# mvenouziou/Boosted_DETR

Hardware: AMD Instinct MI355X
Metric: images/sec training step (fwd+matcher+loss+bwd), 640x640 N=100 (higher is better)
Workload: dtype f32 (conv/GEMM products as 3 split-f16 [fwd] / split-bf16 [grad] MFMA products, f32 accumulate)

## Files before the change

boosted_detr_amd/_lib.py:

```python
from __future__ import annotations

import ctypes as C
import os
from pathlib import Path

_LIB_PATH = Path(os.environ.get("BDETR_LIB") or Path(__file__).resolve().parent / "csrc" / "libbdetr.so")
_lib = None

c_f32p = C.c_void_p
c_i32p = C.c_void_p
c_i64p = C.c_void_p
c_stream = C.c_void_p


class ConvDesc(C.Structure):
    _fields_ = [(n, C.c_int) for n in ("N", "H", "W", "C", "K", "R", "S", "stride", "pad", "OH", "OW")]


class GemmDesc(C.Structure):
    _fields_ = [
        ("I", C.c_int), ("J", C.c_int), ("R", C.c_int), ("nb0", C.c_int), ("nb1", C.c_int),
        ("a", C.c_void_p), ("lda", C.c_int64), ("sa0", C.c_int64), ("sa1", C.c_int64), ("a_rcontig", C.c_int),
        ("b", C.c_void_p), ("ldb", C.c_int64), ("sb0", C.c_int64), ("sb1", C.c_int64), ("b_rcontig", C.c_int),
        ("c", C.c_void_p), ("ldc", C.c_int64), ("sc0", C.c_int64), ("sc1", C.c_int64),
# ... 60 lines not shown
    "bdetr_jpeg_quality_ws_bytes": (C.c_int64, [I, I, I]),
    "bdetr_jpeg_quality": (I, [P, P, P, I, I, I, P, P]),
    "bdetr_augment_jpeg": (I, [P, P, P, P, P, I, I, I, P, P, P]),
    "bdetr_conv2d_fwd": (I, [P, P, P, P, C.POINTER(ConvDesc), I, P, P, P]),
    "bdetr_conv2d_fwd_stat_chunks": (I, [C.POINTER(ConvDesc)]),
    "bdetr_conv2d_bwd_data": (I, [P, P, P, C.POINTER(ConvDesc), I, P]),
    "bdetr_conv2d_bwd_weight": (I, [P, P, P, C.POINTER(ConvDesc), I, P]),
    "bdetr_conv2d_bwd_weight_splitk": (I, [C.POINTER(ConvDesc)]),
    "bdetr_bn_apply_p16": (I, [P, P, P, P, P, P, I, C.POINTER(BnAffine), I, P, P, P, P, P, L, I, P]),
    "bdetr_bn_bwd_p16": (I, [P, P, I, P, P, P, P, P, I, I, P, P, P, P, P, P, P, P, I, L, I, P]),
    "bdetr_bn_bwd_p16_even_pixels": (I, [P, P, I, P, P, P, P, P, I, I, P, P, P, P, P, P, I, I, I, I, I, P]),
    "bdetr_p16_supported": (I, [C.POINTER(ConvDesc)]),
    "bdetr_p16_pack": (I, [P, L, P, P, P, P]),
    "bdetr_p16_unpack": (I, [P, I, L, P, P]),
    "bdetr_p16_pack_conv_weights": (I, [P, I, I, I, I, P, P, P, P]),
    "bdetr_p16_pack_conv_weights_multi": (I, [P, I, P, P]),
    "bdetr_p16_conv2d_fwd_stat_chunks": (I, [C.POINTER(ConvDesc)]),
    "bdetr_p16_conv2d_fwd": (I, [P, P, P, P, C.POINTER(ConvDesc), I, P, P, P]),
    "bdetr_p16_conv2d_bwd_data": (I, [P, P, P, C.POINTER(ConvDesc), I, P]),
    "bdetr_p16_conv2d_bwd_data_stat_chunks": (I, [C.POINTER(ConvDesc)]),
    "bdetr_p16_conv2d_bwd_data_masked_accum": (I, [P, P, P, P, C.POINTER(ConvDesc), C.POINTER(BnBwdFuse), P]),
    "bdetr_p16_conv2d_bwd_data_masked_accum_compact": (I, [P, P, P, P, P, C.POINTER(ConvDesc), C.POINTER(BnBwdFuse), P]),
    "bdetr_relu_mask_apply": (I, [P, P, C.c_int64, P]),
    "bdetr_p16_conv2d_bwd_data_bnstats": (I, [P, P, P, C.POINTER(ConvDesc), C.POINTER(BnBwdFuse), P]),
    "bdetr_p16_conv2d_bwd_weight_splitk": (I, [C.POINTER(ConvDesc)]),
    "bdetr_p16_conv2d_bwd_weight": (I, [P, P, P, C.POINTER(ConvDesc), I, P]),
    "bdetr_p16_conv2d_bwd_weight_xf16": (I, [P, P, P, C.POINTER(ConvDesc), I, P]),
    "bdetr_gemm": (I, [C.POINTER(GemmDesc), P]),
    "bdetr_gemm_ws": (I, [C.POINTER(GemmDesc), P, L, P]),
    "bdetr_splitk_workspace_elems": (L, [L, L, I]),
    "bdetr_conv2d_bwd_weight_ws": (I, [P, P, P, C.POINTER(ConvDesc), I, P, L, P]),
    "bdetr_p16_conv2d_bwd_weight_ws": (I, [P, I, P, P, C.POINTER(ConvDesc), I, P, L, P]),
    "bdetr_gemm_grouped": (I, [C.POINTER(GemmDesc), I, P]),
    "bdetr_colsum_chunks": (I, [L]),
    "bdetr_colsum": (I, [P, L, I, P, P, P]),
    "bdetr_colsum_accumulate": (I, [P, L, I, P, P]),
    "bdetr_colsum_accumulate_group": (I, [P, P, I, P, I, P]),
    "bdetr_colstats": (I, [P, L, I, P, P, P]),
    "bdetr_bn_stats": (I, [P, L, I, P, P, I, F, F, I, P, P, P, P, P, P, P]),
    "bdetr_flag_nonfinite": (I, [P, L, P, P]),
    "bdetr_flag_snapshot": (I, [P, P, P, I, P]),
    "bdetr_debug_checksum": (I, [P, L, P, P, P, I, U64, P]),
    "bdetr_graph_node_census": (I, [P, P, I]),
    "bdetr_bn_stats_fold_rows": (I, []),
    "bdetr_bn_stats_frozen": (I, [P, P, I, F, P, P, P]),
    "bdetr_bn_apply": (I, [P, P, P, P, P, P, I, P, L, I, P]),
    "bdetr_bn_bwd_chunks": (I, [L]),
    "bdetr_bn_bwd": (I, [P, P, P, P, P, P, P, I, I, P, P, P, P, P, L, I, P]),
    "bdetr_maxpool3x3s2_fwd": (I, [P, P, I, I, I, I, I, I, P]),
    "bdetr_maxpool3x3s2_bwd": (I, [P, P, P, P, I, I, I, I, I, I, P]),
    "bdetr_stem_pool_bwd_chunks": (I, [L]),
    "bdetr_stem_pool_fwd": (I, [P, P, P, P, P, I, I, I, I, P, P, P, P, P]),
    "bdetr_stem_pool_bwd": (I, [P, P, P, P, P, P, P, I, I, I, I, P, I, P, P, P, P]),
    "bdetr_p16_s2d_pack_bf16": (I, [P, I, I, I, P, P]),
    "bdetr_p16_stem_bwd_weight": (I, [P, P, P, I, I, I, I, P]),
    "bdetr_p16_s2d_unpack_dw": (I, [P, P, I, P]),
    "bdetr_attention_head_dim": (I, []),
    "bdetr_attention_fwd": (I, [P, P, P, P, P, I, I, I, I, F, P]),
    "bdetr_attention_bwd": (I, [P, P, P, P, P, P, P, P, P, P, I, I, I, I, F, P]),
    "bdetr_softmax_rows_fwd": (I, [P, P, L, I, F, P]),
    "bdetr_softmax_rows_bwd": (I, [P, P, P, L, I, F, P]),
    "bdetr_add_dropout_layernorm_fwd": (I, [P, P, P, P, P, P, P, L, I, F, F, U64, P, P]),
    "bdetr_ln_bwd_chunks": (I, [L]),
    "bdetr_add_dropout_layernorm_bwd": (I, [P, P, P, P, P, P, P, P, P, P, P, L, I, F, U64, P, I, P]),
    "bdetr_rowchain_fwd": (I, [C.POINTER(RowchainFwdDesc), P]),
    "bdetr_rowchain_bwd": (I, [C.POINTER(RowchainBwdDesc), P]),
# ... 74 lines not shown
```

boosted_detr_amd/csrc/igemm.hip:

```cpp
#include "gemm_common.h"
#include <stdlib.h>
#include <string.h>
#include <type_traits>
#include <utility>
#include <vector>

using namespace bdgemm;

namespace {

constexpr int BK = 32;
constexpr int RPAD = 4;
constexpr int NTHREADS = 256;

constexpr int SLD = 36;
constexpr int SLD3 = 52;
constexpr float LO_SCALE = 2048.f;
typedef __bf16 bf16x2 __attribute__((ext_vector_type(2)));
typedef __bf16 bf16x8 __attribute__((ext_vector_type(8)));
typedef _Float16 f16x2 __attribute__((ext_vector_type(2)));
typedef _Float16 f16x8 __attribute__((ext_vector_type(8)));
typedef float f32x2 __attribute__((ext_vector_type(2)));

template <int ARITH>
// ... 43 lines not shown
__device__ __forceinline__ f32x4 buf_load4(__amdgpu_buffer_rsrc_t r, unsigned byte_off) {
    return __builtin_bit_cast(f32x4, __builtin_amdgcn_raw_buffer_load_b128(r, (int)byte_off, 0, 0));
}
__device__ __forceinline__ float buf_load1(__amdgpu_buffer_rsrc_t r, unsigned byte_off) {
    return __builtin_bit_cast(float, __builtin_amdgcn_raw_buffer_load_b32(r, (int)byte_off, 0, 0));
}

template <int VEC>
struct DenseLoader {
    using Op = DenseOp;
    struct Ctx { unsigned off; bool ok; };
    static __device__ __forceinline__ const float* batch_base(const Op& op, int b0, int b1) {
        return op.p + (int64_t)b0 * op.s0 + (int64_t)b1 * op.s1;
    }
    static __device__ __forceinline__ void regroup(Op& op, const float* p, int x_extent, bool rc) {
        op.p = p;
        if (x_extent >= 0) { if (rc) op.rows = x_extent; else op.cols = x_extent; }
    }
    static __device__ __forceinline__ Ctx row_ctx(const Op& op, int row, int row_limit) {
        Ctx c; c.ok = row < row_limit; c.off = (unsigned)row * (unsigned)op.ld; return c;
    }
    static __device__ __forceinline__ f32x4 load(__amdgpu_buffer_rsrc_t rs, const Op& op, const Ctx& c, int col, int col_limit) {
        if (VEC == 4) {
            return buf_load4(rs, (c.ok && col < col_limit) ? (c.off + (unsigned)col) * 4u : OOB);
        } else {
            f32x4 v;
#pragma unroll
            for (int e = 0; e < 4; ++e) v[e] = buf_load1(rs, (c.ok && col + e < col_limit) ? (c.off + (unsigned)(col + e)) * 4u : OOB);
            return v;
        }
    }
};

struct PatchLoader {
    using Op = PatchOp;
    struct Ctx { int nbase; int ih0, iw0; bool ok; };
    static __device__ __forceinline__ const float* batch_base(const Op& op, int, int) { return op.p; }
    static __device__ __forceinline__ void regroup(Op&, const float*, int, bool) {}
    static __device__ __forceinline__ Ctx row_ctx(const Op& op, int row, int row_limit) {
        Ctx c; c.ok = row < row_limit;
        int ohw = op.OH * op.OW;
        int n = row / ohw; int rem = row - n * ohw;
        int oh = rem / op.OW; int ow = rem - oh * op.OW;
        c.nbase = n * op.H * op.W;
        c.ih0 = oh * op.stride - op.pad; c.iw0 = ow * op.stride - op.pad;
        return c;
    }
    static __device__ __forceinline__ f32x4 load(__amdgpu_buffer_rsrc_t rs, const Op& op, const Ctx& c, int col, int col_limit) {
        int tap = col / op.C; int ch = col - tap * op.C;
        int r = tap / op.S; int s = tap - r * op.S;
        int ih = c.ih0 + r, iw = c.iw0 + s;
        const bool ok = c.ok && col < col_limit && (unsigned)ih < (unsigned)op.H && (unsigned)iw < (unsigned)op.W;
        const unsigned off = ((unsigned)(c.nbase + ih * op.W + iw) * (unsigned)op.C + (unsigned)ch) * 4u;
        return buf_load4(rs, ok ? off : OOB);
    }
};

struct WFlipLoader {
    using Op = WFlipOp;
    struct Ctx { unsigned off; bool ok; };
    static __device__ __forceinline__ const float* batch_base(const Op& op, int, int) { return op.p; }
    static __device__ __forceinline__ void regroup(Op&, const float*, int, bool) {}
    static __device__ __forceinline__ Ctx row_ctx(const Op& op, int row, int row_limit) {
        Ctx c; c.ok = row < row_limit;
        int tap = row / op.K; int k = row - tap * op.K;
        int r = tap / op.S; int s = tap - r * op.S;
        c.off = (unsigned)(((k * op.R + (op.R - 1 - r)) * op.S + (op.S - 1 - s)) * op.C);
        return c;
    }
    static __device__ __forceinline__ f32x4 load(__amdgpu_buffer_rsrc_t rs, const Op& op, const Ctx& c, int col, int col_limit) {
        return buf_load4(rs, (c.ok && col < col_limit) ? (c.off + (unsigned)col) * 4u : OOB);
    }
};

template <int BX, bool RC>
struct TileGeom {
    static constexpr int LDS_FLOATS = RC ? BX * (BK + RPAD) : BK * BX;
    static constexpr int NV = BX * BK / 4 / NTHREADS;
    static constexpr int VPR = RC ? BK / 4 : BX / 4;
    static constexpr int LDS_LD = RC ? BK + RPAD : BX;
};

template <int BM, int BN, int WM, int WN, class LA, bool A_RC, class LB, bool B_RC, int ARITH>
__global__ __launch_bounds__(NTHREADS, 2)
void igemm_kernel(typename LA::Op opa, typename LB::Op opb, GemmParams g)
{
    static_assert(WM * WN == 4, "4 waves per workgroup");
    constexpr int WTM = BM / WM, WTN = BN / WN;
    constexpr int TM = WTM / 32, TN = WTN / 32;
    static_assert(TM >= 1 && TN >= 1, "wave tile must hold at least one 32x32 MFMA tile");
    using GA = TileGeom<BM, A_RC>;
    using GB = TileGeom<BN, B_RC>;
    static_assert(GA::NV >= 1 && GB::NV >= 1, "tile too small for 256 threads");

    constexpr bool SPLIT = ARITH != AR_FP32;
    constexpr bool X6 = ARITH == AR_BF16X6;
    constexpr int SLDK = X6 ? SLD3 : SLD;
    constexpr int A_FLOATS = SPLIT ? BM * SLDK : GA::LDS_FLOATS;
    constexpr int B_FLOATS = SPLIT ? BN * SLDK : GB::LDS_FLOATS;
    constexpr int STAGE_FLOATS = A_FLOATS + B_FLOATS;
    static_assert(!SPLIT || ((A_RC || GA::NV % 2 == 0) && (B_RC || GB::NV % 2 == 0)), "split mode transposes k-pairs");
    __shared__ __attribute__((aligned(16))) float lds[2 * STAGE_FLOATS];

    const int tid = threadIdx.x;
    const int lane = tid & 63;
    const int wave = tid >> 6;
    const int wm = wave / WN, wn = wave % WN;
    const int li = lane & 31, lh = lane >> 5;

    const int nwg_ = g.tiles_i * g.tiles_j;
    const bool sk_ = g.ngroups == 0 && g.splitk > 1;
    const int lin_ = sk_ ? xcd_tile(blockIdx.z * nwg_ + blockIdx.x, nwg_ * gridDim.z) : xcd_tile(blockIdx.x, nwg_);
    const int zz_ = sk_ ? lin_ / nwg_ : blockIdx.z;
    const int wg = sk_ ? lin_ - zz_ * nwg_ : lin_;
    const int tile_i = wg / g.tiles_j, tile_j = wg - tile_i * g.tiles_j;
    const int i0 = tile_i * BM, j0 = tile_j * BN;

    int b0 = 0, b1 = 0, r_begin = 0, r_end = g.R;
    if (g.ngroups > 0) {
        const int z = g.splitk > 1 ? (int)blockIdx.z / g.splitk : (int)blockIdx.z;
        if (g.splitk > 1) {
            r_begin = ((int)blockIdx.z - z * g.splitk) * g.r_chunk;
            r_end = min(g.R, r_begin + g.r_chunk);
        }
#define BDETR_PICK(arr) (z == 0 ? g.arr[0] : z == 1 ? g.arr[1] : z == 2 ? g.arr[2] : g.arr[3])
        g.I = BDETR_PICK(gI); g.c = BDETR_PICK(gc); g.bias = BDETR_PICK(gbias);
        const float* pa = BDETR_PICK(ga);
        const float* pb = BDETR_PICK(gb);
#undef BDETR_PICK
        if (i0 >= g.I) return;
        LA::regroup(opa, pa, g.I, A_RC);
        LB::regroup(opb, pb, -1, B_RC);
    } else if (g.splitk > 1) {
        r_begin = zz_ * g.r_chunk;
        r_end = min(g.R, r_begin + g.r_chunk);
    } else {
        b0 = blockIdx.z / g.nb1; b1 = blockIdx.z - b0 * g.nb1;
    }
    const __amdgpu_buffer_rsrc_t rsA = make_rsrc(LA::batch_base(opa, b0, b1));
    const __amdgpu_buffer_rsrc_t rsB = make_rsrc(LB::batch_base(opb, b0, b1));
    const int a_rows = A_RC ? opa.rows : min(opa.rows, r_end), a_cols = A_RC ? min(opa.cols, r_end) : opa.cols;
    const int b_rows = B_RC ? opb.rows : min(opb.rows, r_end), b_cols = B_RC ? min(opb.cols, r_end) : opb.cols;

    typename LA::Ctx ctxA[GA::NV];
    typename LB::Ctx ctxB[GB::NV];
    int colA[GA::NV], colB[GB::NV], ldsoffA[GA::NV], ldsoffB[GB::NV], rowA[GA::NV], rowB[GB::NV];
    auto stage_geom = [&](int p, int vpr, int bx, bool rc, int lds_ld, int& row, int& col, int& ldsoff) {
        if (!SPLIT) {
            const int v = tid + NTHREADS * p;
            const int rt = v / vpr, c4 = v - rt * vpr;
            row = rt; col = 4 * c4; ldsoff = rt * lds_ld + 4 * c4;
        } else if (rc) {
            const int v = tid + NTHREADS * p;
            const int q = v / vpr, c4 = v - q * vpr;
            const int rt = (q & ~15) | ((q & 3) << 2) | ((q >> 2) & 3);
            row = rt; col = 4 * c4;
            ldsoff = rt * SLDK * 32 + ((((c4 >> 1) ^ ((rt >> 4) & 7)) << 2) | ((c4 & 1) << 1));
        } else {
            const int u = tid + NTHREADS * (p >> 1);
            const int kp = u / (bx / 4), c4 = u - kp * (bx / 4);
            row = 2 * kp + (p & 1); col = 4 * c4;
            ldsoff = (4 * c4) * SLDK * 32 + ((((kp >> 2) ^ ((c4 >> 2) & 7)) << 2) | (kp & 3));
        }
    };
#pragma unroll
    for (int p = 0; p < GA::NV; ++p) {
        stage_geom(p, GA::VPR, BM, A_RC, GA::LDS_LD, rowA[p], colA[p], ldsoffA[p]);
        if (A_RC) ctxA[p] = LA::row_ctx(opa, i0 + rowA[p], a_rows);
    }
#pragma unroll
    for (int p = 0; p < GB::NV; ++p) {
        stage_geom(p, GB::VPR, BN, B_RC, GB::LDS_LD, rowB[p], colB[p], ldsoffB[p]);
        if (B_RC) ctxB[p] = LB::row_ctx(opb, j0 + rowB[p], b_rows);
    }

    f32x4 stA0[GA::NV], stB0[GB::NV], stA1[GA::NV], stB1[GB::NV];
    auto load_stage = [&](int r0, f32x4 (&ra)[GA::NV], f32x4 (&rb)[GB::NV]) {
#pragma unroll
        for (int p = 0; p < GA::NV; ++p) {
            if (A_RC) ra[p] = LA::load(rsA, opa, ctxA[p], r0 + colA[p], a_cols);
            else      ra[p] = LA::load(rsA, opa, LA::row_ctx(opa, r0 + rowA[p], a_rows), i0 + colA[p], a_cols);
        }
#pragma unroll
        for (int p = 0; p < GB::NV; ++p) {
            if (B_RC) rb[p] = LB::load(rsB, opb, ctxB[p], r0 + colB[p], b_cols);
            else      rb[p] = LB::load(rsB, opb, LB::row_ctx(opb, r0 + rowB[p], b_rows), j0 + colB[p], b_cols);
        }
    };
    auto write_split = [&](unsigned* base, bool rc, auto nv_c, const f32x4* r, const int* ldsoff) {
        constexpr int nv = decltype(nv_c)::value;
        if (rc) {
#pragma unroll
            for (int p = 0; p < nv; ++p) {
                unsigned* row = base + (ldsoff[p] >> 5);
                const int w = ldsoff[p] & 31;
                if constexpr (X6) {
                    unsigned h0, m0, l0, h1, m1, l1;
                    split3(r[p][0], r[p][1], h0, m0, l0);
                    split3(r[p][2], r[p][3], h1, m1, l1);
                    u32x2 hi, mid, lo;
                    hi[0] = h0; hi[1] = h1; mid[0] = m0; mid[1] = m1; lo[0] = l0; lo[1] = l1;
                    *reinterpret_cast<u32x2*>(row + w) = hi;
                    *reinterpret_cast<u32x2*>(row + (w ^ 16)) = mid;
                    *reinterpret_cast<u32x2*>(row + 32 + (w & 15)) = lo;
                } else {
                    unsigned h0, l0, h1, l1;
                    split2<ARITH>(r[p][0], r[p][1], h0, l0);
                    split2<ARITH>(r[p][2], r[p][3], h1, l1);
                    u32x2 hi, lo;
                    hi[0] = h0; hi[1] = h1; lo[0] = l0; lo[1] = l1;
                    *reinterpret_cast<u32x2*>(row + w) = hi;
                    *reinterpret_cast<u32x2*>(row + (w ^ 16)) = lo;
                }
            }
        } else {
#pragma unroll
            for (int p = 0; p + 1 < nv; p += 2) {
                unsigned* row = base + (ldsoff[p] >> 5);
                const int w = ldsoff[p] & 31;
// ... 235 lines not shown
    }
    if (tiles(128, 128) >= 16LL * num_cus() && J >= 1024) return {128, 128};
    return {64, 64};
}

struct ProfRec { hipEvent_t e0, e1; double flops; int I, J, R, z, bm, bn, kind; };
std::vector<ProfRec> g_prof_recs;
std::vector<std::pair<hipEvent_t, hipEvent_t>> g_prof_pool;
size_t g_prof_used = 0;

template <class L> struct LoaderId { static constexpr int v = 0; };
template <> struct LoaderId<PatchLoader> { static constexpr int v = 1; };
template <> struct LoaderId<WFlipLoader> { static constexpr int v = 2; };
template <> struct LoaderId<DenseLoader<1>> { static constexpr int v = 3; };

}
namespace bdgemm {
bool g_prof_on = false;
void prof_begin(hipStream_t st, double flops, int I, int J, int R, int z, int bm, int bn, int kind) {
    if (g_prof_used == g_prof_pool.size()) {
        hipEvent_t a, b;
        if (hipEventCreate(&a) != hipSuccess || hipEventCreate(&b) != hipSuccess) return;
        g_prof_pool.emplace_back(a, b);
    }
    auto& ev = g_prof_pool[g_prof_used++];
    g_prof_recs.push_back({ev.first, ev.second, flops, I, J, R, z, bm, bn, kind});
    (void)hipEventRecord(ev.first, st);
}
void prof_end(hipStream_t st) { (void)hipEventRecord(g_prof_recs.back().e1, st); }
}
namespace {

template <int BM, int BN, int WM, int WN, class LA, bool A_RC, class LB, bool B_RC, int ARITH = AR_FP32>
int launch_cfg(const typename LA::Op& a, const typename LB::Op& b, GemmParams g, int zdim, hipStream_t st) {
    g.tiles_i = (int)cdiv64(g.I, BM);
    g.tiles_j = (int)cdiv64(g.J, BN);
    dim3 grid(g.tiles_i * g.tiles_j, 1, zdim);
    g.vec_store = (g.J % 4 == 0) && (g.ldc % 4 == 0) && (g.sc0 % 4 == 0) && (g.sc1 % 4 == 0) && ((reinterpret_cast<uintptr_t>(g.c) & 15) == 0);
    const bool prof = g_prof_on;
    if (prof) prof_begin(st, 2.0 * (double)g.I * (double)g.J * (double)g.R * (g.splitk > 1 ? (g.ngroups > 0 ? (double)g.ngroups : 1.0) : (double)zdim), g.I, g.J, g.R, zdim, BM, BN,
                         ARITH * 10000 + LoaderId<LA>::v * 1000 + (A_RC ? 100 : 0) + LoaderId<LB>::v * 10 + (B_RC ? 1 : 0));
    hipLaunchKernelGGL((igemm_kernel<BM, BN, WM, WN, LA, A_RC, LB, B_RC, ARITH>), grid, dim3(NTHREADS), 0, st, a, b, g);
    if (prof) prof_end(st);
    return bdetr_launch_status("igemm");
}

template <class LA, bool A_RC, class LB, bool B_RC>
int launch_any(const typename LA::Op& a, const typename LB::Op& b, GemmParams g, int zdim, hipStream_t st, int arith, bool small_only = false) {
    if (arith == AR_FP16X3 && !(A_RC && B_RC)) arith = AR_FP32;
    constexpr bool PATCH = LoaderId<LA>::v == 1 || LoaderId<LB>::v == 1;
    TileChoice t = small_only ? TileChoice{64, 64} : choose_tile(g.I, g.J, g.splitk > 1 ? 2 : zdim, A_RC && B_RC, arith != AR_FP32, PATCH);
    if constexpr (LoaderId<LA>::v != 3 && LoaderId<LB>::v != 3) {
        if (arith == AR_BF16X3 && t.bn >= 64) {
            if (t.bm == 128 && t.bn == 128) return launch_cfg<128, 128, 2, 2, LA, A_RC, LB, B_RC, AR_BF16X3>(a, b, g, zdim, st);
            if (t.bm == 128 && t.bn == 64)  return launch_cfg<128, 64, 2, 2, LA, A_RC, LB, B_RC, AR_BF16X3>(a, b, g, zdim, st);
            return launch_cfg<64, 64, 2, 2, LA, A_RC, LB, B_RC, AR_BF16X3>(a, b, g, zdim, st);
        }
        if (arith == AR_BF16X6 && t.bn >= 64) {
            if (t.bm == 128) return launch_cfg<128, 64, 2, 2, LA, A_RC, LB, B_RC, AR_BF16X6>(a, b, g, zdim, st);
            return launch_cfg<64, 64, 2, 2, LA, A_RC, LB, B_RC, AR_BF16X6>(a, b, g, zdim, st);
        }
        if constexpr (A_RC && B_RC) {
            if (arith == AR_FP16X3 && t.bn >= 64) {
                if (t.bm == 128 && t.bn == 128) return launch_cfg<128, 128, 2, 2, LA, A_RC, LB, B_RC, AR_FP16X3>(a, b, g, zdim, st);
                if (t.bm == 128 && t.bn == 64)  return launch_cfg<128, 64, 2, 2, LA, A_RC, LB, B_RC, AR_FP16X3>(a, b, g, zdim, st);
                return launch_cfg<64, 64, 2, 2, LA, A_RC, LB, B_RC, AR_FP16X3>(a, b, g, zdim, st);
            }
        }
    }
    if (t.bm == 128 && t.bn == 128) return launch_cfg<128, 128, 2, 2, LA, A_RC, LB, B_RC>(a, b, g, zdim, st);
    if (t.bm == 128 && t.bn == 64)  return launch_cfg<128, 64, 2, 2, LA, A_RC, LB, B_RC>(a, b, g, zdim, st);
    if (t.bm == 128 && t.bn == 32)  return launch_cfg<128, 32, 4, 1, LA, A_RC, LB, B_RC>(a, b, g, zdim, st);
    return launch_cfg<64, 64, 2, 2, LA, A_RC, LB, B_RC>(a, b, g, zdim, st);
// ... 105 lines not shown
        BDETR_CHECK_ARG(span_ok((int64_t)(e.a_rcontig ? e.I : e.R) * e.lda) && span_ok((int64_t)(e.b_rcontig ? e.J : e.R) * e.ldb),
                        "bdetr_gemm_grouped: operand %d spans 4 GB or more (32-bit buffer offsets)", k);
        g.ga[k] = e.a; g.gb[k] = e.b; g.gc[k] = e.c; g.gbias[k] = e.bias; g.gI[k] = e.I;
        if (e.I > maxI) maxI = e.I;
        v4 = v4 && aligned16(e.a) && aligned16(e.b) && aligned16(e.c);
    }
    const bdetr_gemm_desc& f = d[0];
    bool dims4 = f.J % 4 == 0 && (f.a_rcontig || f.b_rcontig ? f.R % 4 == 0 : true);
    for (int k = 0; k < n; ++k) dims4 = dims4 && (f.a_rcontig || d[k].I % 4 == 0);
    BDETR_CHECK_ARG(v4 && f.lda % 4 == 0 && f.ldb % 4 == 0 && f.ldc % 4 == 0 && dims4,
                    "bdetr_gemm_grouped: operands must be 16-byte aligned with contiguous dimensions that are multiples of 4");
    g.ngroups = n;
    g.I = maxI; g.J = f.J; g.R = f.R;
    g.c = f.c; g.ldc = f.ldc; g.bias = f.bias; g.alpha = f.alpha; g.act = f.act;
    g.mode = f.accumulate ? ST_ACCUM : ST_STORE;
    int zdim = n;
    if (f.splitk > 1) {
        g.r_chunk = (int)(cdiv64(cdiv64(f.R, f.splitk), BK) * BK);
        g.splitk = (int)cdiv64(f.R, g.r_chunk);
        g.mode = ST_ATOMIC;
        zdim = n * g.splitk;
    }
    DenseOp a{f.a, f.lda, 0, 0, f.a_rcontig ? maxI : f.R, f.a_rcontig ? f.R : maxI};
    DenseOp b{f.b, f.ldb, 0, 0, f.b_rcontig ? f.J : f.R, f.b_rcontig ? f.R : f.J};
    hipStream_t st = (hipStream_t)stream;
    const bool arc = f.a_rcontig != 0, brc = f.b_rcontig != 0;
    const int sp = use_split(f.grad != 0);
    if (arc && brc)   return launch_any<DenseLoader<4>, true, DenseLoader<4>, true>(a, b, g, zdim, st, sp);
    if (arc && !brc)  return launch_any<DenseLoader<4>, true, DenseLoader<4>, false>(a, b, g, zdim, st, sp);
    if (!arc && !brc) return launch_any<DenseLoader<4>, false, DenseLoader<4>, false>(a, b, g, zdim, st, sp);
    return launch_any<DenseLoader<4>, false, DenseLoader<4>, true>(a, b, g, zdim, st, sp, true);
}

extern "C" int bdetr_gemm(const bdetr_gemm_desc* d, void* stream) { return bdetr_gemm_ws(d, nullptr, 0, stream); }

template <class F>
static int with_splitk_slabs(GemmParams& g, int zdim, float* ws, int64_t ws_elems, hipStream_t st, const char* who, F&& launch) {
    float* c = g.c;
    const int64_t n = (int64_t)g.I * g.J, slab = splitk_slab(n);
    BDETR_CHECK_ARG(g.ldc == g.J, "%s: the split-K workspace form needs a dense C (ldc == J)", who);
    BDETR_CHECK_ARG(aligned16(ws) && ws_elems >= (int64_t)zdim * slab, "%s: workspace too small or misaligned (%lld floats, need %lld)", who,
                    (long long)ws_elems, (long long)((int64_t)zdim * slab));
    g.c = ws; g.sc0 = slab; g.mode = ST_STORE;
    if (int e = launch()) return e;
    return splitk_fold(ws, zdim, slab, c, n, st);
}

extern "C" int bdetr_gemm_ws(const bdetr_gemm_desc* d, float* ws, int64_t ws_elems, void* stream) {
    BDETR_CHECK_ARG(d && d->a && d->b && d->c, "bdetr_gemm: null pointer");
    BDETR_CHECK_ARG(d->I > 0 && d->J > 0 && d->R >= 0, "bdetr_gemm: bad shape I=%d J=%d R=%d", d->I, d->J, d->R);
    const int nb0 = d->nb0 > 0 ? d->nb0 : 1, nb1 = d->nb1 > 0 ? d->nb1 : 1;
    const int splitk = d->splitk > 1 ? d->splitk : 1;
    BDETR_CHECK_ARG(splitk == 1 || (nb0 * nb1 == 1 && !d->bias && d->act == 0), "bdetr_gemm: splitk needs a single plain GEMM");
    hipStream_t st = (hipStream_t)stream;

    DenseOp a{d->a, d->lda, d->sa0, d->sa1, d->a_rcontig ? d->I : d->R, d->a_rcontig ? d->R : d->I};
    DenseOp b{d->b, d->ldb, d->sb0, d->sb1, d->b_rcontig ? d->J : d->R, d->b_rcontig ? d->R : d->J};
    BDETR_CHECK_ARG(span_ok(dense_span(a)) && span_ok(dense_span(b)),
                    "bdetr_gemm: an operand matrix spans 4 GB or more (32-bit buffer offsets); split the problem");
    GemmParams g; init_params(g);
    g.I = d->I; g.J = d->J; g.R = d->R; g.nb1 = nb1;
    g.c = d->c; g.ldc = d->ldc; g.sc0 = d->sc0; g.sc1 = d->sc1;
    g.bias = d->bias; g.alpha = d->alpha; g.act = d->act;
    g.mode = splitk > 1 ? ST_ATOMIC : (d->accumulate ? ST_ACCUM : ST_STORE);
    int zdim = nb0 * nb1;
    if (splitk > 1) {
// ... 162 lines not shown
```

boosted_detr_amd/engine.py:

```python
from __future__ import annotations

import math
import zlib
from typing import Callable, Dict, List, Optional, Sequence

import numpy as np
import torch

from . import kernels as K

_DEVICE = None


def device() -> torch.device:
    global _DEVICE
    if _DEVICE is None:
        if not torch.cuda.is_available():
            raise RuntimeError("boosted_detr_amd needs an AMD GPU (HIP device); there is no CPU execution path")
        _DEVICE = torch.device("cuda", torch.cuda.current_device())
    return _DEVICE


def to_device(a, dtype=torch.float32) -> torch.Tensor:
    if isinstance(a, torch.Tensor):
# ... 176 lines not shown
        K.relu_mask_apply_(g, r.lazy_mask)
        r.lazy_mask = None
    return g


class Tape:

    def __init__(self):
        self.nodes: List[tuple] = []

    def record(self, outputs: Sequence[torch.Tensor], inputs: Sequence[Optional[torch.Tensor]], fn: Callable) -> None:
        self.nodes.append((tuple(outputs), tuple(inputs), fn))

    def backward(self, seeds: Dict[int, torch.Tensor]) -> Dict[int, torch.Tensor]:
        grads: Dict[int, torch.Tensor] = dict(seeds)
        for outputs, inputs, fn in reversed(self.nodes):
            gouts = [grads.pop(id(o), None) for o in outputs]
            if all(g is None for g in gouts):
                continue
            if not getattr(fn, "accepts_lazy", False):
                gouts = [materialise(g) for g in gouts]
            acc = None
            if getattr(fn, "wants_acc", False):
                acc = []
                for t in inputs:
                    have = grads.get(id(t)) if t is not None else None
                    acc.append(have if info(have).owned else None)
                gins = fn(*gouts, acc=acc)
            else:
                gins = fn(*gouts)
            if not isinstance(gins, (tuple, list)):
                gins = (gins,)
            assert len(gins) == len(inputs), (len(gins), len(inputs))
            for i, (t, g) in enumerate(zip(inputs, gins)):
                if t is None or g is None:
                    continue
                key = id(t)
                if key in grads:
                    if acc is not None and acc[i] is not None and g is acc[i]:
                        grads[key] = g
                        continue
                    g, have = materialise(g), materialise(grads[key])
                    dense_contribution(have)
                    if info(have).owned:
                        K.axpy_(1.0, g.view(have.shape), have)
                        grads[key] = have
                    else:
                        grads[key] = own(K.add(have, g.view(have.shape)))
                else:
                    grads[key] = g
            if _CAPTURE[0] is not None:
                _CAPTURE[0].maybe_cut(next((g for g in gins if isinstance(g, torch.Tensor)), None) if _DEBUG_LOG[0] is not None else None)
            elif _DEBUG_LOG[0] is not None and _DEBUG_LOG[0].eager_pending >= SegmentedCapture.SIDE_TASKS_PER_SEGMENT:
                _debug_cut(next((g for g in gins if isinstance(g, torch.Tensor)), None))
        return grads


_TAPE: Optional[Tape] = None
_CAPTURE = [None]


def capture() -> Optional["SegmentedCapture"]:
    return _CAPTURE[0]


def set_capture(cap: Optional["SegmentedCapture"]) -> None:
    _CAPTURE[0] = cap

import os as _os

# ... 451 lines not shown
```

boosted_detr_amd/kernels.py:

```python
from __future__ import annotations

import ctypes as C
from dataclasses import dataclass
from typing import Optional, Tuple

import numpy as np
import torch

from . import _lib
from ._lib import BnAffine, BnBwdFuse, ConvDesc, GemmDesc, LossDesc, RowchainBwdDesc, RowchainFwdDesc, check

ACT_NONE, ACT_RELU, ACT_TANH = 0, 1, 2


_LAUNCH_STREAM = [None]


def set_launch_stream(handle: Optional[int]) -> Optional[int]:
    prev = _LAUNCH_STREAM[0]
    _LAUNCH_STREAM[0] = handle
    return prev


GEMM_FP32, GEMM_BF16X3, GEMM_MIXED, GEMM_SPLIT, GEMM_BF16X6 = 0, 1, 2, 3, 4
# ... 423 lines not shown
def gemm_raw(I, J, R, a, lda, a_rc, b, ldb, b_rc, c, ldc, *, nb0=1, nb1=1, sa=(0, 0), sb=(0, 0), sc=(0, 0),
             bias=None, alpha=1.0, act=ACT_NONE, accumulate=False, splitk=1, grad=False):
    _chk(a, b, c, bias)
    g = GemmDesc(I, J, R, nb0, nb1, _p(a), lda, sa[0], sa[1], int(a_rc), _p(b), ldb, sb[0], sb[1], int(b_rc),
                 _p(c), ldc, sc[0], sc[1], _p(bias), float(alpha), act, int(accumulate), splitk, int(grad))
    ws, n = _splitk_ws(I, J, splitk, c) if ldc == J else (None, 0)
    check(_lib.lib().bdetr_gemm_ws(C.byref(g), _p(ws), n, _stream()), "gemm")
    return c


def gemm_grouped(descs):
    arr = (GemmDesc * len(descs))()
    for k, (I, J, R, a, lda, a_rc, b, ldb, b_rc, c, ldc, bias, act, acc) in enumerate(descs):
        _chk(a, b, c, bias)
        arr[k] = GemmDesc(I, J, R, 1, 1, _p(a), lda, 0, 0, int(a_rc), _p(b), ldb, 0, 0, int(b_rc), _p(c), ldc, 0, 0, _p(bias), 1.0, act,
                          int(acc), 1, int(not (a_rc and b_rc)))
    check(_lib.lib().bdetr_gemm_grouped(arr, len(descs), _stream()), "gemm_grouped")


def linear_fwd_group(xs, ws, biases, act=ACT_NONE):
    K_, O = xs[0].shape[1], ws[0].shape[0]
    ys = [empty(x.shape[0], O, like=x) for x in xs]
    gemm_grouped([(x.shape[0], O, K_, x, K_, True, w, K_, True, y, O, b, act, False) for x, w, b, y in zip(xs, ws, biases, ys)])
    return ys


def linear_bwd_data_group(dys, ws):
    O, K_ = ws[0].shape
    dxs = [empty(dy.shape[0], K_, like=dy) for dy in dys]
    gemm_grouped([(dy.shape[0], K_, O, dy, O, True, w, K_, False, dx, K_, None, ACT_NONE, False) for dy, w, dx in zip(dys, ws, dxs)])
    return dxs


def linear_fwd(x2d, w, bias, act=ACT_NONE):
    M, K = x2d.shape
    O = w.shape[0]
    y = empty(M, O, like=x2d)
    return gemm_raw(M, O, K, x2d, K, True, w, K, True, y, O, bias=bias, act=act)


def linear_bwd_data(dy2d, w, dx=None, accumulate=False):
    M, O = dy2d.shape
    K = w.shape[1]
    if dx is None:
        dx = empty(M, K, like=dy2d)
    return gemm_raw(M, K, O, dy2d, O, True, w, K, False, dx, K, accumulate=accumulate, grad=True)


def _auto_splitk(I, J, R) -> int:
    cus = _lib.lib().bdetr_device_cus()
    tiles = max(1, ((I + 63) // 64) * ((J + 63) // 64))
    sk = max(1, min((2 * cus) // tiles, R // 128))
    return sk


def linear_bwd_weight(dy2d, x2d, dw=None, prezeroed: bool = False):
    M, O = dy2d.shape
    K = x2d.shape[1]
    if dw is None:
        dw = empty(O, K, like=dy2d)
        prezeroed = False
    sk = _auto_splitk(O, K, M)
    if sk > 1 and not prezeroed:
        check(_lib.lib().bdetr_zero(_p(dw), dw.numel(), _stream()), "zero")
    return gemm_raw(O, K, M, dy2d, O, False, x2d, K, False, dw, K, splitk=sk, grad=True)

# ... 513 lines not shown
```

boosted_detr_amd/ops.py:

```python
from __future__ import annotations

import math
import os
import weakref
from typing import Optional

import numpy as np
import torch

from . import kernels as K
from . import _lib
from .engine import WEIGHTS_VERSION, Variable, current_tape, dense_contribution, info, materialise, own, side_task, tag

_dropout_site = [0]
_dropout_seed_dev = [None]


def dropout_seed_tensor() -> torch.Tensor:
    if _dropout_seed_dev[0] is None:
        _dropout_seed_dev[0] = torch.full((1,), 0x5EED, dtype=torch.int64, device="cuda")
    return _dropout_seed_dev[0]


def set_dropout_seed(seed: int, write: bool = True) -> None:
# ... 472 lines not shown
            _param_grads_task(w, b, lambda dw, pz: K.stem_bwd_weight_s2d(x32, dy, dw), None, x32, dy)
        else:
            _param_grads_task(w, b, lambda dw, pz: K.conv2d_bwd_weight(x32, dy, g, dw=dw, prezeroed=pz), None, x32, dy)
        return (None,)

    _rec([out], [x], backward)
    return out


def dense(x: torch.Tensor, w: Variable, b: Variable, act: int = K.ACT_NONE) -> torch.Tensor:
    x2d = _2d(x)
    y2d = K.linear_fwd(x2d, w.value, b.value, act)
    y = y2d.view(*x.shape[:-1], w.value.shape[0])

    def backward(g_out, acc=None):
        g2d = _2d(g_out.contiguous())
        if act == K.ACT_RELU:
            g2d = K.relu_bwd(y2d, g2d)
        elif act == K.ACT_TANH:
            g2d = K.tanh_bwd(y2d, g2d)
        _param_grads_task(w, b, lambda dw, pz: K.linear_bwd_weight(g2d, x2d, dw=dw, prezeroed=pz), g2d, x2d, g2d)
        have = acc[0] if acc is not None else None
        if have is not None and have.is_contiguous() and have.shape == x.shape:
            K.linear_bwd_data(g2d, w.value, dx=_2d(materialise(have)), accumulate=True)
            dense_contribution(have)
            return (have,)
        return (own(K.linear_bwd_data(g2d, w.value).view(x.shape)),)

    backward.wants_acc = True
    _rec([y], [x], backward)
    return y


def dense_group(xs, ws, bs):
    x2 = [_2d(x) for x in xs]
    aligned = all(t.data_ptr() % 16 == 0 for t in x2) and x2[0].shape[1] % 4 == 0 and ws[0].value.shape[0] % 4 == 0
    same = all(w.value.shape == ws[0].value.shape for w in ws)
    if not (aligned and same) or len(xs) > 4:
        return [dense(x, w, b) for x, w, b in zip(xs, ws, bs)]
    y2 = K.linear_fwd_group(x2, [w.value for w in ws], [b.value for b in bs])
    ys = [y.view(*x.shape[:-1], y.shape[1]) for y, x in zip(y2, xs)]

    def backward(*gs):
        g2 = [_2d(g.contiguous()) for g in gs]

        def param_grads():
            groups = {}
            for g, x, w in zip(g2, x2, ws):
                if w.needs_grad:
                    groups.setdefault((tuple(g.shape), tuple(x.shape)), []).append((g, x, GradSink(w)))
            for members in groups.values():
                K.linear_bwd_weight_group([m[0] for m in members], [m[1] for m in members], [m[2].buf for m in members], [m[2].mode == "direct" for m in members])
                for m in members:
                    m[2].commit()
            sinks = [(g, GradSink(b)) for g, b in zip(g2, bs) if b.needs_grad]
            direct = [(g, s) for g, s in sinks if s.mode == "direct"]
            if len(direct) > 1 and not K.deterministic() and all(g.shape[1] == direct[0][0].shape[1] for g, _ in direct):
                K.colsum_group([g for g, _ in direct], [s.buf for _, s in direct])
                for _, s in direct:
                    s.commit()
                sinks = [(g, s) for g, s in sinks if s.mode != "direct"]
            for g, s in sinks:
                K.colsum(g, out=s.buf, prezeroed=s.mode == "direct")
                s.commit()
        if any(w.needs_grad or b.needs_grad for w, b in zip(ws, bs)):
            side_task(param_grads, *x2, *g2)
        dxs = K.linear_bwd_data_group(g2, [w.value for w in ws])
        return tuple(own(dx.view(x.shape)) for dx, x in zip(dxs, xs))

    _rec(ys, list(xs), backward)
    return ys


def add(a: torch.Tensor, b: torch.Tensor) -> torch.Tensor:
    out = K.add(a, b)
    _rec([out], [a, b], lambda g: (g, g))
    return out


def _param_or_tensor_grad(p, fn):
    if isinstance(p, Variable):
        if p.needs_grad:
            s = GradSink(p)
            fn(s.buf)
            s.commit()
        return None
    return fn(None)


def add_bcast(x: torch.Tensor, row) -> torch.Tensor:
    rv = row.value if isinstance(row, Variable) else row
    out = K.add_bcast_rows(x, rv)
    n = rv.numel()

    def backward(g):
        g = g.contiguous()
        grow = _param_or_tensor_grad(row, lambda out_: K.sum_over_batch(g, n, out=out_))
        return g, (grow.view(rv.shape) if grow is not None else None)

    _rec([out], [x, None if isinstance(row, Variable) else row], backward)
    return out

# ... 193 lines not shown
```

include/bdetr.h:

```cpp
#ifndef BDETR_H
#define BDETR_H
#include <stdint.h>
#ifdef __cplusplus
extern "C" {
#endif

#define BDETR_ABI_VERSION 8

int         bdetr_abi_version(void);
const char* bdetr_last_error(void);
int         bdetr_device_cus(void);

int         bdetr_low_priority_stream_create(void** stream_out);
int         bdetr_stream_priority_range(int* least, int* greatest);
int         bdetr_side_stream_candidates(void* main_stream, int ncand, int loads, int ticks, void** streams_out, float* scores_ms, float* unloaded_ms);
int         bdetr_stream_destroy(void* stream);

enum { BDETR_GEMM_FP32 = 0, BDETR_GEMM_BF16X3 = 1, BDETR_GEMM_MIXED = 2, BDETR_GEMM_SPLIT = 3, BDETR_GEMM_BF16X6 = 4 };
int         bdetr_set_gemm_precision(int mode);
int         bdetr_get_gemm_precision(void);

int bdetr_prof_enable(int on);
int bdetr_prof_read(double* total_ms, int64_t* launches, double* flops);
int bdetr_prof_read_arith(int arith, double* total_ms, int64_t* launches, double* flops);
// ... 62 lines not shown
    const float* y; const float* mean; const float* rstd; const float* gamma; const float* beta; int relu;
    float* part_g; float* part_gx;
    const uint64_t* relu_mask;
    const float* y2; const float* mean2; const float* rstd2; float* part_gx2;
} bdetr_bn_bwd_fuse;
int bdetr_p16_conv2d_bwd_data_stat_chunks(const bdetr_conv_desc* d);
int bdetr_relu_mask_apply(float* x, const uint64_t* relu_mask, int64_t n, void* stream);
int bdetr_p16_conv2d_bwd_data_masked_accum(const void* dy_bf16, const void* wt_bf16, float* dx, const uint64_t* relu_mask,
                                           const bdetr_conv_desc* d, const bdetr_bn_bwd_fuse* bn , void* stream);
int bdetr_p16_conv2d_bwd_data_masked_accum_compact(const void* dy_bf16, const void* wt_bf16, float* dx, const float* old_even,
                                                   const uint64_t* relu_mask, const bdetr_conv_desc* d, const bdetr_bn_bwd_fuse* bn, void* stream);
int bdetr_p16_conv2d_bwd_data_bnstats(const void* dy_bf16, const void* wt_bf16, float* dx,
                                      const bdetr_conv_desc* d, const bdetr_bn_bwd_fuse* bn, void* stream);
int bdetr_p16_conv2d_bwd_weight_splitk(const bdetr_conv_desc* d);
int bdetr_p16_conv2d_bwd_weight(const void* x_bf16, const void* dy_bf16, float* dw,
                                const bdetr_conv_desc* d, int splitk, void* stream);
int bdetr_p16_conv2d_bwd_weight_xf16(const void* x_f16, const void* dy_bf16, float* dw,
                                     const bdetr_conv_desc* d, int splitk, void* stream);
int bdetr_p16_conv2d_bwd_weight_ws(const void* x, int x_is_f16, const void* dy_bf16, float* dw,
                                   const bdetr_conv_desc* d, int splitk, float* ws, int64_t ws_elems, void* stream);

typedef struct {
    int I, J, R;
    int nb0, nb1;
    const float* a; int64_t lda, sa0, sa1; int a_rcontig;
    const float* b; int64_t ldb, sb0, sb1; int b_rcontig;
    float*       c; int64_t ldc, sc0, sc1;
    const float* bias; float alpha; int act; int accumulate; int splitk;
    int grad;
} bdetr_gemm_desc;
int bdetr_gemm(const bdetr_gemm_desc* g, void* stream);
int bdetr_gemm_ws(const bdetr_gemm_desc* g, float* ws, int64_t ws_elems, void* stream);
int bdetr_gemm_grouped(const bdetr_gemm_desc* g, int n, void* stream);

int bdetr_colsum_chunks(int64_t rows);
int bdetr_colsum(const float* x, int64_t rows, int cols, float* out, float* ws, void* stream);
int bdetr_colsum_accumulate(const float* x, int64_t rows, int cols, float* out, void* stream);
int bdetr_colsum_accumulate_group(const float* const* xs, const int64_t* rows, int cols, float* const* outs, int n, void* stream);

int bdetr_colstats(const float* x, int64_t rows, int C, float* part_sum, float* part_sq, void* stream);
int bdetr_bn_stats(const float* x, int64_t rows, int C, const float* part_sum, const float* part_sq,
                   int nparts, float eps, float momentum, int bessel,
                   float* mean, float* rstd, float* moving_mean, float* moving_var, float* fold_ws,
                   int* guard_flag, void* stream);
int bdetr_flag_nonfinite(const float* x, int64_t n, int* flag, void* stream);
int bdetr_flag_snapshot(const int* flag, int* ordinal, int* host_ring, int ring_len, void* stream);
int bdetr_debug_checksum(const float* x, int64_t n, uint64_t* scratch, uint64_t* log, int* cursor, int cap, uint64_t tag, void* stream);
int bdetr_graph_node_census(void* graph, int64_t* counts, int ncounts);
int bdetr_bn_stats_fold_rows(void);
int bdetr_bn_stats_frozen(const float* moving_mean, const float* moving_var, int C, float eps,
                          float* mean, float* rstd, void* stream);
int bdetr_bn_apply(const float* x, const float* mean, const float* rstd, const float* gamma,
                   const float* beta, const float* residual, int relu, float* out,
                   int64_t rows, int C, void* stream);
int bdetr_bn_bwd_chunks(int64_t rows);
int bdetr_bn_bwd(const float* dout, const float* out, const float* x, const float* mean,
                 const float* rstd, const float* gamma, const float* beta, int relu, int frozen,
                 float* dx, float* dgamma, float* dbeta, float* dresidual,
                 float* ws, int64_t rows, int C, void* stream);

int bdetr_maxpool3x3s2_fwd(const float* x, float* y, int N, int H, int W, int C, int OH, int OW, void* stream);
int bdetr_maxpool3x3s2_bwd(const float* x, const float* y, const float* dy, float* dx,
                           int N, int H, int W, int C, int OH, int OW, void* stream);

int bdetr_stem_pool_bwd_chunks(int64_t rows);
int bdetr_stem_pool_fwd(const float* y, const float* mean, const float* rstd, const float* gamma, const float* beta,
// ... 128 lines not shown
```

Measured before the change: 649.0.

## Fuse fan-in linear backward-data products into one K-chained GEMM per destination

Adds a K-chained GEMM loader that walks several (dy, W) pairs in sequence inside one kernel, so the input gradients of a dense group whose members share an input are summed in the accumulator. The result can also be written straight into an existing gradient buffer. This removes the separate per-member backward-data GEMMs, the intermediate dx tensors and the elementwise gradient additions done by the autograd engine. The engine learns to skip re-adding aliased gradients the backward has already summed. It adds complexity in the GEMM kernel and the autograd path, and is bypassed in deterministic mode.

```diff
diff --git a/boosted_detr_amd/_lib.py b/boosted_detr_amd/_lib.py
--- a/boosted_detr_amd/_lib.py
+++ b/boosted_detr_amd/_lib.py
@@ -116,6 +116,7 @@
     "bdetr_conv2d_bwd_weight_ws": (I, [P, P, P, C.POINTER(ConvDesc), I, P, L, P]),
     "bdetr_p16_conv2d_bwd_weight_ws": (I, [P, I, P, P, C.POINTER(ConvDesc), I, P, L, P]),
     "bdetr_gemm_grouped": (I, [C.POINTER(GemmDesc), I, P]),
+    "bdetr_linear_bwd_data_fanin": (I, [P, P, P, P, I, I, I, I, I, P]),
     "bdetr_colsum_chunks": (I, [L]),
     "bdetr_colsum": (I, [P, L, I, P, P, P]),
     "bdetr_colsum_accumulate": (I, [P, L, I, P, P]),
diff --git a/boosted_detr_amd/csrc/igemm.hip b/boosted_detr_amd/csrc/igemm.hip
--- a/boosted_detr_amd/csrc/igemm.hip
+++ b/boosted_detr_amd/csrc/igemm.hip
@@ -99,6 +99,27 @@
     }
 };
 
+constexpr int CHAIN_MAX = 12;
+struct ChainOp { const float* p[CHAIN_MAX]; int64_t ld; int rows, cols; int n[2], rm, acc; };
+struct ChainLoader {
+    using Op = ChainOp;
+    using Ctx = DenseLoader<4>::Ctx;
+    static constexpr bool CHAINED = true;
+    static __device__ __forceinline__ const float* member(const Op& op, int m) { return op.p[m]; }
+    static __device__ __forceinline__ int first(const Op& op, int z) { return z == 0 ? 0 : op.n[0]; }
+    static __device__ __forceinline__ int count(const Op& op, int z) { return z == 0 ? op.n[0] : op.n[1]; }
+    static __device__ __forceinline__ const float* batch_base(const Op& op, int z, int) { return op.p[first(op, z)]; }
+    static __device__ __forceinline__ void regroup(Op&, const float*, int, bool) {}
+    static __device__ __forceinline__ Ctx row_ctx(const Op& op, int row, int row_limit) {
+        Ctx c; c.ok = row < row_limit; c.off = (unsigned)row * (unsigned)op.ld; return c;
+    }
+    static __device__ __forceinline__ f32x4 load(__amdgpu_buffer_rsrc_t rs, const Op&, const Ctx& c, int col, int col_limit) {
+        return buf_load4(rs, (c.ok && col < col_limit) ? (c.off + (unsigned)col) * 4u : OOB);
+    }
+};
+template <class L, class = void> struct IsChained { static constexpr bool v = false; };
+template <class L> struct IsChained<L, std::enable_if_t<L::CHAINED>> { static constexpr bool v = true; };
+
 struct PatchLoader {
     using Op = PatchOp;
     struct Ctx { int nbase; int ih0, iw0; bool ok; };
@@ -162,6 +183,8 @@
 
     constexpr bool SPLIT = ARITH != AR_FP32;
     constexpr bool X6 = ARITH == AR_BF16X6;
+    constexpr bool CHAIN = IsChained<LA>::v;
+    static_assert(CHAIN == IsChained<LB>::v, "both operands of a K-chained product are chained");
     constexpr int SLDK = X6 ? SLD3 : SLD;
     constexpr int A_FLOATS = SPLIT ? BM * SLDK : GA::LDS_FLOATS;
     constexpr int B_FLOATS = SPLIT ? BN * SLDK : GB::LDS_FLOATS;
@@ -204,8 +227,16 @@
     } else {
         b0 = blockIdx.z / g.nb1; b1 = blockIdx.z - b0 * g.nb1;
     }
-    const __amdgpu_buffer_rsrc_t rsA = make_rsrc(LA::batch_base(opa, b0, b1));
-    const __amdgpu_buffer_rsrc_t rsB = make_rsrc(LB::batch_base(opb, b0, b1));
+    __amdgpu_buffer_rsrc_t rsA = make_rsrc(LA::batch_base(opa, b0, b1));
+    __amdgpu_buffer_rsrc_t rsB = make_rsrc(LB::batch_base(opb, b0, b1));
+    [[maybe_unused]] int ch_m = 0, ch_r = 0;
+    [[maybe_unused]] int ch_n = 1, ch_first = 0;
+    if constexpr (CHAIN) {
+        g.c = b0 == 0 ? g.gc[0] : g.gc[1];
+        g.mode = ((opa.acc >> b0) & 1) ? ST_ACCUM : ST_STORE;
+        ch_n = LA::count(opa, b0); ch_first = LA::first(opa, b0);
+        r_end = ch_n * opa.rm;
+    }
     const int a_rows = A_RC ? opa.rows : min(opa.rows, r_end), a_cols = A_RC ? min(opa.cols, r_end) : opa.cols;
     const int b_rows = B_RC ? opb.rows : min(opb.rows, r_end), b_cols = B_RC ? min(opb.cols, r_end) : opb.cols;
 
@@ -243,6 +274,7 @@
 
     f32x4 stA0[GA::NV], stB0[GB::NV], stA1[GA::NV], stB1[GB::NV];
     auto load_stage = [&](int r0, f32x4 (&ra)[GA::NV], f32x4 (&rb)[GB::NV]) {
+        if constexpr (CHAIN) r0 = ch_r;
 #pragma unroll
         for (int p = 0; p < GA::NV; ++p) {
             if (A_RC) ra[p] = LA::load(rsA, opa, ctxA[p], r0 + colA[p], a_cols);
@@ -252,6 +284,14 @@
         for (int p = 0; p < GB::NV; ++p) {
             if (B_RC) rb[p] = LB::load(rsB, opb, ctxB[p], r0 + colB[p], b_cols);
             else      rb[p] = LB::load(rsB, opb, LB::row_ctx(opb, r0 + rowB[p], b_rows), j0 + colB[p], b_cols);
+        }
+        if constexpr (CHAIN) {
+            ch_r += BK;
+            if (ch_r >= opa.rm && ch_m + 1 < ch_n) {
+                ++ch_m; ch_r = 0;
+                rsA = make_rsrc(LA::member(opa, ch_first + ch_m));
+                rsB = make_rsrc(LB::member(opb, ch_first + ch_m));
+            }
         }
     };
     auto write_split = [&](unsigned* base, bool rc, auto nv_c, const f32x4* r, const int* ldsoff) {
@@ -553,13 +593,14 @@
 namespace {
 
 template <int BM, int BN, int WM, int WN, class LA, bool A_RC, class LB, bool B_RC, int ARITH = AR_FP32>
-int launch_cfg(const typename LA::Op& a, const typename LB::Op& b, GemmParams g, int zdim, hipStream_t st) {
+int launch_cfg(const typename LA::Op& a, const typename LB::Op& b, GemmParams g, int zdim, hipStream_t st, double prof_flops = -1.0, int prof_R = 0) {
     g.tiles_i = (int)cdiv64(g.I, BM);
     g.tiles_j = (int)cdiv64(g.J, BN);
     dim3 grid(g.tiles_i * g.tiles_j, 1, zdim);
     g.vec_store = (g.J % 4 == 0) && (g.ldc % 4 == 0) && (g.sc0 % 4 == 0) && (g.sc1 % 4 == 0) && ((reinterpret_cast<uintptr_t>(g.c) & 15) == 0);
     const bool prof = g_prof_on;
-    if (prof) prof_begin(st, 2.0 * (double)g.I * (double)g.J * (double)g.R * (g.splitk > 1 ? (g.ngroups > 0 ? (double)g.ngroups : 1.0) : (double)zdim), g.I, g.J, g.R, zdim, BM, BN,
+    if (prof && prof_flops >= 0.0) prof_begin(st, prof_flops, g.I, g.J, prof_R, 1, BM, BN, ARITH * 10000 + (A_RC ? 100 : 0) + (B_RC ? 1 : 0));
+    else if (prof) prof_begin(st, 2.0 * (double)g.I * (double)g.J * (double)g.R * (g.splitk > 1 ? (g.ngroups > 0 ? (double)g.ngroups : 1.0) : (double)zdim), g.I, g.J, g.R, zdim, BM, BN,
                          ARITH * 10000 + LoaderId<LA>::v * 1000 + (A_RC ? 100 : 0) + LoaderId<LB>::v * 10 + (B_RC ? 1 : 0));
     hipLaunchKernelGGL((igemm_kernel<BM, BN, WM, WN, LA, A_RC, LB, B_RC, ARITH>), grid, dim3(NTHREADS), 0, st, a, b, g);
     if (prof) prof_end(st);
@@ -731,6 +772,45 @@
     return launch_any<DenseLoader<4>, false, DenseLoader<4>, true>(a, b, g, zdim, st, sp, true);
 }
 
+extern "C" int bdetr_linear_bwd_data_fanin(const float* const* gs, const float* const* ws, float* const* dxs, const int* nmem, int ndst,
+                                           int I, int J, int R, int acc_bits, void* stream) {
+    BDETR_CHECK_ARG(gs && ws && dxs && nmem && ndst >= 1 && ndst <= 2, "bdetr_linear_bwd_data_fanin: 1..2 destinations");
+    int total = 0, longest = 0;
+    for (int z = 0; z < ndst; ++z) {
+        BDETR_CHECK_ARG(nmem[z] >= 1 && nmem[z] <= 6, "bdetr_linear_bwd_data_fanin: destination %d has %d members (1..6)", z, nmem[z]);
+        total += nmem[z];
+        if (nmem[z] > longest) longest = nmem[z];
+    }
+    static_assert(CHAIN_MAX >= 2 * 6, "two destinations of six members");
+    BDETR_CHECK_ARG(I > 0 && J > 0 && R > 0 && J % 4 == 0 && R % BK == 0,
+                    "bdetr_linear_bwd_data_fanin: bad shape I=%d J=%d R=%d (J a multiple of 4, R a multiple of %d)", I, J, R, BK);
+    BDETR_CHECK_ARG(span_ok((int64_t)I * R) && span_ok((int64_t)R * J),
+                    "bdetr_linear_bwd_data_fanin: an operand spans 4 GB or more (32-bit buffer offsets)");
+    ChainOp a{}, b{};
+    for (int k = 0; k < total; ++k) {
+        BDETR_CHECK_ARG(gs[k] && ws[k] && aligned16(gs[k]) && aligned16(ws[k]), "bdetr_linear_bwd_data_fanin: member %d is null or not 16-byte aligned", k);
+        a.p[k] = gs[k]; b.p[k] = ws[k];
+    }
+    GemmParams g; init_params(g);
+    for (int z = 0; z < ndst; ++z) {
+        BDETR_CHECK_ARG(dxs[z] && aligned16(dxs[z]), "bdetr_linear_bwd_data_fanin: destination %d is null or not 16-byte aligned", z);
+        g.gc[z] = dxs[z];
+        a.n[z] = b.n[z] = nmem[z];
+    }
+    a.ld = R; a.rows = I; a.cols = R; a.rm = R; a.acc = acc_bits;
+    b.ld = J; b.rows = R; b.cols = J; b.rm = R; b.acc = acc_bits;
+    g.I = I; g.J = J; g.R = longest * R;
+    g.c = dxs[0]; g.ldc = J;
+    hipStream_t st = (hipStream_t)stream;
+    const double flops = 2.0 * (double)I * (double)J * (double)R * (double)total;
+    if (J <= 32) return launch_cfg<128, 32, 4, 1, ChainLoader, true, ChainLoader, false>(a, b, g, ndst, st, flops, total * R);
+    switch (use_split(true)) {
+        case AR_BF16X3: return launch_cfg<64, 64, 2, 2, ChainLoader, true, ChainLoader, false, AR_BF16X3>(a, b, g, ndst, st, flops, total * R);
+        case AR_BF16X6: return launch_cfg<64, 64, 2, 2, ChainLoader, true, ChainLoader, false, AR_BF16X6>(a, b, g, ndst, st, flops, total * R);
+        default:        return launch_cfg<64, 64, 2, 2, ChainLoader, true, ChainLoader, false>(a, b, g, ndst, st, flops, total * R);
+    }
+}
+
 extern "C" int bdetr_gemm(const bdetr_gemm_desc* d, void* stream) { return bdetr_gemm_ws(d, nullptr, 0, stream); }
 
 template <class F>
diff --git a/boosted_detr_amd/engine.py b/boosted_detr_amd/engine.py
--- a/boosted_detr_amd/engine.py
+++ b/boosted_detr_amd/engine.py
@@ -232,10 +232,15 @@
             if not isinstance(gins, (tuple, list)):
                 gins = (gins,)
             assert len(gins) == len(inputs), (len(gins), len(inputs))
+            summed = {} if getattr(fn, "sums_aliases", False) else None
             for i, (t, g) in enumerate(zip(inputs, gins)):
                 if t is None or g is None:
                     continue
                 key = id(t)
+                if summed is not None:
+                    if summed.get(key) is g:
+                        continue
+                    summed[key] = g
                 if key in grads:
                     if acc is not None and acc[i] is not None and g is acc[i]:
                         grads[key] = g
diff --git a/boosted_detr_amd/kernels.py b/boosted_detr_amd/kernels.py
--- a/boosted_detr_amd/kernels.py
+++ b/boosted_detr_amd/kernels.py
@@ -479,6 +479,33 @@
     return dxs
 
 
+FANIN_MAX_MEMBERS, FANIN_MAX_DESTS = 6, 2
+
+
+def fanin_applies(dys, ws) -> bool:
+    O, K_ = ws[0].shape
+    return (O % 32 == 0 and K_ % 4 == 0 and all(w.shape == ws[0].shape and w.is_contiguous() and w.data_ptr() % 16 == 0 for w in ws)
+            and all(dy.shape == dys[0].shape and dy.is_contiguous() and dy.data_ptr() % 16 == 0 for dy in dys))
+
+
+def linear_bwd_data_fanin(dests):
+    assert 1 <= len(dests) <= FANIN_MAX_DESTS and all(1 <= len(d[0]) <= FANIN_MAX_MEMBERS and len(d[0]) == len(d[1]) for d in dests)
+    M, O = dests[0][0][0].shape
+    K_ = dests[0][1][0].shape[1]
+    gs = [g for d in dests for g in d[0]]
+    ws = [w for d in dests for w in d[1]]
+    assert all(g.shape == (M, O) for g in gs) and all(w.shape == (O, K_) for w in ws)
+    assert all(d[2] is not None or not d[3] for d in dests)
+    dxs = [d[2] if d[2] is not None else empty(M, K_, like=gs[0]) for d in dests]
+    assert all(dx.shape == (M, K_) for dx in dxs)
+    _chk(*gs, *ws, *dxs)
+    PA, PD, NA = C.c_void_p * len(gs), C.c_void_p * len(dxs), C.c_int * len(dxs)
+    acc_bits = sum(1 << z for z, d in enumerate(dests) if d[3])
+    check(_lib.lib().bdetr_linear_bwd_data_fanin(PA(*[g.data_ptr() for g in gs]), PA(*[w.data_ptr() for w in ws]), PD(*[dx.data_ptr() for dx in dxs]),
+                                                 NA(*[len(d[0]) for d in dests]), len(dxs), M, K_, O, acc_bits, _stream()), "linear_bwd_data_fanin")
+    return dxs
+
+
 def linear_fwd(x2d, w, bias, act=ACT_NONE):
     M, K = x2d.shape
     O = w.shape[0]
diff --git a/boosted_detr_amd/ops.py b/boosted_detr_amd/ops.py
--- a/boosted_detr_amd/ops.py
+++ b/boosted_detr_amd/ops.py
@@ -528,6 +528,44 @@
     return y
 
 
+FANIN = os.environ.get("BDETR_FANIN", "1") != "0"
+
+
+def _dense_group_fanin(xs, g2, wv, acc):
+    if not FANIN or K.deterministic() or not K.fanin_applies(g2[:1], wv):
+        return None
+    dests = {}
+    for i, x in enumerate(xs):
+        d = dests.setdefault(id(x), [[], None])
+        d[0].append(i)
+        have = acc[i] if acc is not None else None
+        if have is not None and have.is_contiguous() and have.shape == x.shape and info(have).compact_even is None:
+            d[1] = have
+    if len(dests) == len(xs) and all(d[1] is None for d in dests.values()):
+        return None
+    by_rows = {}
+    for d in dests.values():
+        if len(d[0]) > K.FANIN_MAX_MEMBERS or not K.fanin_applies([g2[i] for i in d[0]], wv):
+            return None
+        by_rows.setdefault(g2[d[0][0]].shape[0], []).append(d)
+    out = [None] * len(xs)
+    for group in by_rows.values():
+        for k in range(0, len(group), K.FANIN_MAX_DESTS):
+            part = group[k:k + K.FANIN_MAX_DESTS]
+            haves = [None if d[1] is None else materialise(d[1]) for d in part]
+            dxs = K.linear_bwd_data_fanin([([g2[i] for i in d[0]], [wv[i] for i in d[0]], None if h is None else _2d(h), h is not None)
+                                           for d, h in zip(part, haves)])
+            for d, h, dx in zip(part, haves, dxs):
+                if h is not None:
+                    dense_contribution(h)
+                    res = h
+                else:
+                    res = own(dx.view(xs[d[0][0]].shape))
+                for i in d[0]:
+                    out[i] = res
+    return tuple(out)
+
+
 def dense_group(xs, ws, bs):
     x2 = [_2d(x) for x in xs]
     aligned = all(t.data_ptr() % 16 == 0 for t in x2) and x2[0].shape[1] % 4 == 0 and ws[0].value.shape[0] % 4 == 0
@@ -537,7 +575,7 @@
     y2 = K.linear_fwd_group(x2, [w.value for w in ws], [b.value for b in bs])
     ys = [y.view(*x.shape[:-1], y.shape[1]) for y, x in zip(y2, xs)]
 
-    def backward(*gs):
+    def backward(*gs, acc=None):
         g2 = [_2d(g.contiguous()) for g in gs]
 
         def param_grads():
@@ -561,9 +599,14 @@
                 s.commit()
         if any(w.needs_grad or b.needs_grad for w, b in zip(ws, bs)):
             side_task(param_grads, *x2, *g2)
+        fan = _dense_group_fanin(xs, g2, [w.value for w in ws], acc)
+        if fan is not None:
+            return fan
         dxs = K.linear_bwd_data_group(g2, [w.value for w in ws])
         return tuple(own(dx.view(x.shape)) for dx, x in zip(dxs, xs))
 
+    backward.wants_acc = True
+    backward.sums_aliases = True
     _rec(ys, list(xs), backward)
     return ys
 
diff --git a/include/bdetr.h b/include/bdetr.h
--- a/include/bdetr.h
+++ b/include/bdetr.h
@@ -118,6 +118,8 @@
 int bdetr_gemm(const bdetr_gemm_desc* g, void* stream);
 int bdetr_gemm_ws(const bdetr_gemm_desc* g, float* ws, int64_t ws_elems, void* stream);
 int bdetr_gemm_grouped(const bdetr_gemm_desc* g, int n, void* stream);
+int bdetr_linear_bwd_data_fanin(const float* const* gs, const float* const* ws, float* const* dxs, const int* nmem, int ndst,
+                                int I, int J, int R, int acc_bits, void* stream);
 
 int bdetr_colsum_chunks(int64_t rows);
 int bdetr_colsum(const float* x, int64_t rows, int cols, float* out, float* ws, void* stream);
```

New measurement: 651.9 (median of 6 runs). No clear change (+0.5%).
